# LambdaLabsML/distributed-training-guide

Hardware: NVIDIA H100
Metric: tokens/sec (device-timed, max over ranks) Llama-2-7B seq 4096 bf16 training (higher is better)
Workload: dtype bf16; 1 GPU; model=meta-llama/Llama-2-7b-hf, global_batch=1, seq_len=4096, parallelism=dp1 (ddp+zero1), optimizer=AdamW, bf16 parameters and states

## Files before the change

distributed_training_guide_b200/csrc/api.h:

```cpp
#pragma once
#include <cuda_runtime.h>
#include <cstdint>

namespace dtg {

unsigned long long launch_count();

enum class NormKind : int { kRms, kLn, kLn2 };
enum class NormRes : int { kNone, kAddBefore, kAddAfter };
constexpr int norm_grad_planes(NormKind k) { return k == NormKind::kRms ? 1 : k == NormKind::kLn ? 2 : 4; }
int norm_max_hidden(NormKind k);
struct NormFwdArgs {
  const void* x;
  const void* r;
  const void* w[2];
  const void* b[2];
  void* y[2];
  void* h;
  float* mean;
  float* rstd;
};
void norm_fwd(NormKind k, NormRes res, const NormFwdArgs& a, int T, int H, float eps, cudaStream_t s);
int norm_bwd_grid(NormKind k, int T, int H);
struct NormBwdArgs {
// ... 49 lines not shown
void adamw_flat(void* p, const void* g, void* m, void* v, long long n, float lr, float beta1, float beta2, float eps,
                float wd, int step, float grad_scale, bool state_fp32, cudaStream_t s);

void gemm_bf16(const void* A, const void* B, void* C, int M, int N, int K, long long lda, long long ldb, long long ldc,
               bool a_kmajor, bool b_kmajor, bool accumulate, int variant, cudaStream_t s, const void* bias = nullptr);

void gemm_fp8(const void* A, const void* B, void* C, int M, int N, int K, long long lda, long long ldb, long long ldc,
              bool a_e5m2, const float* scale_a, const float* scale_b, bool accumulate, int variant, cudaStream_t s,
              const void* bias = nullptr);

int gemm_max_active_clusters(int cg);
void gemm_bf16_dist(int mode, const void* const* a_srcs, const void* const* b_srcs, void* const* c_dsts, int M, int N,
                    int K, long long lda, long long ldb, long long ldc, bool b_kmajor, bool accumulate, int nranks,
                    int rank, int rows_per_peer, cudaStream_t s);

void gemm_bf16_bgather(const void* A, void* full_base, void* C, int M, int N, int K, long long lda, long long ldb,
                       long long ldc, bool b_kmajor, const void* const* shards, long long per_bytes, long long w_off,
                       long long w_bytes, uint32_t* counters, uint32_t target, int chunk_shift, uint32_t* const* pads,
                       int nranks, int rank, uint32_t bar_epoch, cudaStream_t s, const void* bias = nullptr);
void gemm_bf16_ag(const void* const* a_bufs, const void* B, void* C, int M, int N, int K, long long ldb, long long ldc,
                  bool b_kmajor, int nranks, int rank, int rows_per_peer, uint32_t* flags, uint32_t ag_epoch,
                  uint32_t* const* pads, uint32_t bar_epoch, int n_comm, cudaStream_t s, const void* bias = nullptr);

void fp8_amax(const void* x, long long R, int C, long long ld, float* amax, cudaStream_t s);
void fp8_cast_transpose(const void* x, long long ld, int R, int C, bool e5m2, const float* amax, void* out, void* out_t,
                        float* scale_inv, cudaStream_t s);

void attn_fwd(const void* qkv, void* o, float* lse, int B, int S, int nh, int nkv, float scale, cudaStream_t s,
              const int* doc_start = nullptr, int window = 0, int head_dim = 128);
void attn_fwd2(const void* qkv, void* o, float* lse, int B, int S, int nh, int nkv, float scale, cudaStream_t s,
               const int* doc_start = nullptr, int window = 0, int head_dim = 128);
void attn_bwd(const void* qkv, const void* o, const void* d_o, const float* lse, float* delta, float* dq_acc,
              void* dqkv, int B, int S, int nh, int nkv, float scale, int mode, cudaStream_t s,
              const int* doc_start = nullptr, int window = 0, int head_dim = 128);

}
```

distributed_training_guide_b200/csrc/attention_bind.cpp:

```cpp
#include <ATen/cuda/CUDAContext.h>
#include <c10/cuda/CUDAGuard.h>
#include <torch/extension.h>

#include <algorithm>
#include <cmath>
#include <cstdint>
#include <cstdlib>
#include <limits>

#include "api.h"
#include "comm_api.h"

namespace dtg {
namespace {
using torch::Tensor;

void check_heads_scale(int64_t nh, int64_t nkv, double scale) {
  TORCH_CHECK(nh >= 1 && nkv >= 1, "nh and nkv must be >= 1, got nh ", nh, ", nkv ", nkv);
  TORCH_CHECK(nh % nkv == 0, "nh must be a multiple of nkv, got nh ", nh, ", nkv ", nkv);
  const float s = (float)scale;
  TORCH_CHECK(std::isfinite(s) && s > 0.f, "scale must be finite and > 0, got ", scale);
}

bool aligned16(const Tensor& t) { return reinterpret_cast<uintptr_t>(t.data_ptr()) % 16 == 0; }
// ... 48 lines not shown
  return (int)std::min<int64_t>(*window, std::numeric_limits<int>::max());
}

int default_fwd_version() {
  static int v = -1;
  if (v < 0) {
    const char* e = getenv("DTG_ATTN_FWD");
    v = e ? atoi(e) : 2;
    if (v != 1 && v != 2) v = 2;
  }
  return v;
}

std::tuple<Tensor, Tensor> py_attn_fwd(const Tensor& qkv, int64_t nh, int64_t nkv, double scale, int64_t version,
                                       const c10::optional<Tensor>& doc_start, const c10::optional<int64_t>& window,
                                       int64_t head_dim) {
  check_qkv(qkv, nh, nkv, scale, head_dim);
  TORCH_CHECK(version >= 0 && version <= 2, "version must be 0 (default), 1 or 2, got ", version);
  const int* ds = doc_start_ptr(doc_start, qkv);
  const int win = window_arg(window);
  const c10::cuda::CUDAGuard guard(qkv.device());
  const int64_t B = qkv.size(0), S = qkv.size(1);
  Tensor o = torch::empty({B, S, nh, head_dim}, qkv.options());
  Tensor lse = torch::empty({B, nh, S}, qkv.options().dtype(at::kFloat));
  if (version == 0) version = default_fwd_version();
  auto fn = version == 1 ? dtg::attn_fwd : dtg::attn_fwd2;
  fn(qkv.data_ptr(), o.data_ptr(), lse.data_ptr<float>(), (int)B, (int)S, (int)nh, (int)nkv, (float)scale,
     at::cuda::getCurrentCUDAStream().stream(), ds, win, (int)head_dim);
  return {o, lse};
}

Tensor py_attn_bwd(const Tensor& d_o, const Tensor& qkv, const Tensor& o, const Tensor& lse, int64_t nh, int64_t nkv,
                   double scale, const c10::optional<Tensor>& trace, int64_t mode,
                   const c10::optional<Tensor>& doc_start, const c10::optional<int64_t>& window, int64_t head_dim) {
  check_qkv(qkv, nh, nkv, scale, head_dim);
  TORCH_CHECK(mode >= 0 && mode <= 2, "mode must be 0 (default), 1 or 2, got ", mode);
  const int* ds = doc_start_ptr(doc_start, qkv);
  const int win = window_arg(window);
  check_rows(o, "o", qkv, nh, head_dim);
  check_rows(d_o, "d_o", qkv, nh, head_dim);
  check_lse(lse, qkv, nh);
  float* tr = nullptr;
  if (trace.has_value() && trace->defined()) {
    TORCH_CHECK(trace->scalar_type() == at::kLong && trace->numel() >= 1024 && trace->is_contiguous() &&
                    trace->device() == qkv.device(),
                "trace must be a contiguous int64[1024] on the device of qkv");
    tr = reinterpret_cast<float*>(trace->data_ptr<int64_t>());
  }
  const c10::cuda::CUDAGuard guard(qkv.device());
  const int64_t B = qkv.size(0), S = qkv.size(1);
  Tensor dqkv = torch::empty_like(qkv);
  Tensor delta = torch::empty({B, nh, S}, qkv.options().dtype(at::kFloat));
  dtg::attn_bwd(qkv.data_ptr(), o.data_ptr(), d_o.data_ptr(), lse.data_ptr<float>(), delta.data_ptr<float>(), tr,
                dqkv.data_ptr(), (int)B, (int)S, (int)nh, (int)nkv, (float)scale, (int)mode,
                at::cuda::getCurrentCUDAStream().stream(), ds, win, (int)head_dim);
  return dqkv;
}
}

void bind_attention(pybind11::module_& m) {
  m.def("attn_fwd", &py_attn_fwd, pybind11::arg("qkv"), pybind11::arg("nh"), pybind11::arg("nkv"), pybind11::arg("scale"),
        pybind11::arg("version") = 0, pybind11::arg("doc_start") = pybind11::none(),
        pybind11::arg("window") = pybind11::none(), pybind11::arg("head_dim") = 128);
  m.def("attn_bwd", &py_attn_bwd, pybind11::arg("d_o"), pybind11::arg("qkv"), pybind11::arg("o"), pybind11::arg("lse"),
        pybind11::arg("nh"), pybind11::arg("nkv"), pybind11::arg("scale"), pybind11::arg("trace") = pybind11::none(),
        pybind11::arg("mode") = 0,
        pybind11::arg("doc_start") = pybind11::none(), pybind11::arg("window") = pybind11::none(),
        pybind11::arg("head_dim") = 128);
}
}
```

distributed_training_guide_b200/csrc/attention_bwd.cu:

```cuda
#include <cuda.h>

#include <cstdlib>

#include "api.h"
#include "attention_common.cuh"
#include "common.cuh"
#include "gemm_common.cuh"
#include "ptx.cuh"

namespace dtg {
using namespace ptx;

namespace bwd {
constexpr int R_HALF = 128 * 128;
constexpr int C_HALF = 64 * 128;
constexpr int Y_STAGES = 3;
constexpr float LOG2E = 1.4426950408889634f;
constexpr int THREADS = 256;
template <int D>
struct Layout {
  static constexpr int R_TILE = 128 * D * 2;
  static constexpr int C_TILE = 64 * D * 2;
  static constexpr int OFF_R1 = 0, OFF_R2 = R_TILE;
  static constexpr int OFF_Y = 2 * R_TILE;
  static constexpr int OFF_P = OFF_Y + Y_STAGES * 2 * C_TILE;
  static constexpr int OFF_DS = OFF_P + 128 * 128;
  static constexpr int OFF_BAR = OFF_DS + 128 * 128;
  static constexpr int SMEM_BYTES = OFF_BAR + 256 + 1024;
};
}

template <int D>
__global__ void attn_bwd_delta_kernel(const __nv_bfloat16* __restrict__ d_o, const __nv_bfloat16* __restrict__ o,
                                      float* __restrict__ delta, long long rows, int S, int nh) {
  const long long row = (blockIdx.x * (long long)blockDim.x + threadIdx.x) >> 5;
  const int lane = threadIdx.x & 31;
  if (row >= rows) return;
  const __nv_bfloat162* a = reinterpret_cast<const __nv_bfloat162*>(d_o + row * D) + lane * (D / 64);
  const __nv_bfloat162* b = reinterpret_cast<const __nv_bfloat162*>(o + row * D) + lane * (D / 64);
  float acc = 0.f;
#pragma unroll
  for (int i = 0; i < D / 64; ++i) {
    const float2 x = __bfloat1622float2(a[i]), y = __bfloat1622float2(b[i]);
    acc += x.x * y.x + x.y * y.y;
  }
  acc = warp_sum(acc);
  if (lane == 0) {
    const long long tok = row / nh;
    const int h = (int)(row % nh);
    const long long bb = tok / S, ss = tok % S;
    delta[(bb * nh + h) * S + ss] = acc;
  }
}

template <bool KV_MODE, bool TS, bool DOC, bool WIN, int D>
__global__ void __launch_bounds__(bwd::THREADS, 1)
attn_bwd_kernel(const __grid_constant__ CUtensorMap tm_qkv_r, const __grid_constant__ CUtensorMap tm_qkv_c,
                const __grid_constant__ CUtensorMap tm_do_r, const __grid_constant__ CUtensorMap tm_do_c,
                const float* __restrict__ lse, const float* __restrict__ delta, __nv_bfloat16* __restrict__ dqkv,
                int S, int nh, int nkv, float scale, int num_r_blocks, long long* __restrict__ trace,
                const int* __restrict__ doc_start, int window) {
  using namespace bwd;
  using L = Layout<D>;
  constexpr int R_TILE = L::R_TILE, C_TILE = L::C_TILE, OFF_R1 = L::OFF_R1, OFF_R2 = L::OFF_R2, OFF_Y = L::OFF_Y,
                OFF_P = L::OFF_P, OFF_DS = L::OFF_DS, OFF_BAR = L::OFF_BAR;
  const bool tracing = trace != nullptr && blockIdx.x == 0 && blockIdx.y == 0;
  extern __shared__ uint8_t smem_raw[];
  uint8_t* smem = reinterpret_cast<uint8_t*>((reinterpret_cast<uintptr_t>(smem_raw) + 1023) & ~uintptr_t(1023));
  uint64_t* bars = reinterpret_cast<uint64_t*>(smem + OFF_BAR);
  uint64_t* res_full = bars + 0;
  uint64_t* y_full = bars + 1;
  uint64_t* y_empty = bars + 5;

  const int warp = threadIdx.x >> 5, lane = threadIdx.x & 31, wg = threadIdx.x >> 7;
  const int group = nh / nkv;
  const int nht = nh + 2 * nkv;
  const int heads_r = KV_MODE ? nkv : nh;
  const int head_r = blockIdx.x % heads_r;
  const int batch = blockIdx.x / heads_r;
  const int r_block = KV_MODE ? (int)blockIdx.y : num_r_blocks - 1 - (int)blockIdx.y;
  const int R0 = r_block * 128;
  const int kv_head = KV_MODE ? head_r : head_r / group;
  int c_start = KV_MODE ? R0 / 64 : 0;
  int n_c = KV_MODE ? (S / 64 - c_start) : (R0 + 128) / 64;
  [[maybe_unused]] const int* ds_row = nullptr;
  [[maybe_unused]] int doc_bound = 0;
  if constexpr (DOC) {
    ds_row = doc_start + (long long)batch * S;
    if (KV_MODE) {
      int lo = c_start, hi = S / 64 - 1;
      while (lo < hi) {
        const int mid = (lo + hi + 1) >> 1;
        if (__ldg(ds_row + mid * 64) <= R0 + 127) lo = mid;
        else hi = mid - 1;
      }
      n_c = lo - c_start + 1;
      hi = c_start + n_c;
      lo = c_start;
      while (lo < hi) {
        const int mid = (lo + hi) >> 1;
        if (__ldg(ds_row + mid * 64 + 63) > R0) hi = mid;
        else lo = mid + 1;
      }
      doc_bound = lo;
    } else {
      c_start = min(max(__ldg(ds_row + R0) / 64, 0), n_c - 1);
      n_c -= c_start;
      doc_bound = __ldg(ds_row + R0 + 127);
    }
  }
  if constexpr (WIN) {
    if (KV_MODE) {
      n_c = min(n_c, min((R0 + 127 + window - 1) / 64, S / 64 - 1) - c_start + 1);
    } else {
      const int c_win = max(R0 - window + 1, 0) / 64;
      if (c_win > c_start) {
        n_c -= c_win - c_start;
        c_start = c_win;
      }
    }
  }
  const int n_iter = KV_MODE ? n_c * group : n_c;

  if (threadIdx.x == 0) {
    prefetch_tensormap(&tm_qkv_r);
    prefetch_tensormap(&tm_qkv_c);
    prefetch_tensormap(&tm_do_r);
    prefetch_tensormap(&tm_do_c);
    mbar_init(res_full, 1);
    for (int i = 0; i < Y_STAGES; ++i) {
      mbar_init(&y_full[i], 1);
      mbar_init(&y_empty[i], 2);
    }
    fence_barrier_init();
  }
  __syncthreads();

  auto issue_y = [&](int t) {
    const int st = t % Y_STAGES;
    const uint32_t ph = (uint32_t)((t / Y_STAGES) & 1);
    const int c = c_start + (KV_MODE ? t % n_c : t);
    const int C0 = c * 64;
    uint8_t* y1 = smem + OFF_Y + st * 2 * C_TILE;
    uint8_t* y2 = y1 + C_TILE;
    mbar_wait_mma(&y_empty[st], ph ^ 1);
    mbar_arrive_expect_tx(&y_full[st], 2 * C_TILE);
    if (KV_MODE) {
      const int qh = kv_head * group + t / n_c;
#pragma unroll
      for (int b = 0; b < D / 64; ++b) tma_load_4d(&tm_qkv_c, &y_full[st], y1 + b * C_HALF, 64 * b, qh, C0, batch);
#pragma unroll
      for (int b = 0; b < D / 64; ++b) tma_load_4d(&tm_do_c, &y_full[st], y2 + b * C_HALF, 64 * b, qh, C0, batch);
    } else {
#pragma unroll
      for (int b = 0; b < D / 64; ++b)
        tma_load_4d(&tm_qkv_c, &y_full[st], y1 + b * C_HALF, 64 * b, nh + kv_head, C0, batch);
#pragma unroll
      for (int b = 0; b < D / 64; ++b)
        tma_load_4d(&tm_qkv_c, &y_full[st], y2 + b * C_HALF, 64 * b, nh + nkv + kv_head, C0, batch);
    }
  };
// ... 42 lines not shown
        const long long idx = ((long long)batch * nh + head_r) * S + R0 + rl0 + 8 * h;
        lse_r[h] = lse[idx] * LOG2E;
        delta_r[h] = delta[idx];
        if constexpr (DOC) ds_r[h] = __ldg(ds_row + R0 + rl0 + 8 * h);
      }
    }
    if constexpr (WIN) {
#pragma unroll
      for (int h = 0; h < 2; ++h) {
        const int idx = R0 + rl0 + 8 * h;
        if constexpr (KV_MODE) ds_r[h] = DOC ? min(ds_r[h], idx + window) : idx + window;
        else ds_r[h] = max(ds_r[h], idx - window + 1);
      }
    }
    [[maybe_unused]] float acc_a[KV_MODE ? D / 2 : 1];
    float acc_b[D / 2];
#pragma unroll
    for (int i = 0; i < D / 2; ++i) {
      if constexpr (KV_MODE) acc_a[i] = 0.f;
      acc_b[i] = 0.f;
    }
    const uint32_t r1 = smem_u32(smem + OFF_R1) + (uint32_t)(half * 8192);
    const uint32_t r2 = smem_u32(smem + OFF_R2) + (uint32_t)(half * 8192);
    const uint32_t sp = smem_u32(smem + OFF_P) + (uint32_t)(half * 8192);
    const uint32_t sds = smem_u32(smem + OFF_DS) + (uint32_t)(half * 8192);
    mbar_wait_mma(res_full, 0);
    for (int t = 0; t < n_iter; ++t) {
      if (threadIdx.x == 0 && t + Y_STAGES - 1 < n_iter) issue_y(t + Y_STAGES - 1);
      const int ys = t % Y_STAGES;
      const int c = c_start + (KV_MODE ? t % n_c : t);
      const int C0 = c * 64;
      [[maybe_unused]] const float* lq = nullptr;
      [[maybe_unused]] const float* dq = nullptr;
      if (KV_MODE) {
        const int qh = kv_head * group + t / n_c;
        lq = lse + ((long long)batch * nh + qh) * S + C0;
        dq = delta + ((long long)batch * nh + qh) * S + C0;
      }
      mbar_wait_mma(&y_full[ys], (uint32_t)((t / Y_STAGES) & 1));
      const uint32_t y1 = smem_u32(smem + OFF_Y + ys * 2 * C_TILE), y2 = y1 + C_TILE;
      float sc[32], dp[32];
#pragma unroll
      for (int i = 0; i < 32; ++i) sc[i] = dp[i] = 0.f;
      wgmma_fence();
      fence_regs(sc);
      fence_regs(dp);
#pragma unroll
      for (int kk = 0; kk < D / 16; ++kk) {
        const uint32_t ra = (uint32_t)((kk >> 2) * R_HALF + (kk & 3) * 32);
        const uint32_t cb = (uint32_t)((kk >> 2) * C_HALF + (kk & 3) * 32);
        wgmma_m64n64k16_ss<0, 0>(sc, desc_kmajor_sw128(r1 + ra), desc_kmajor_sw128(y1 + cb), 1u);
      }
#pragma unroll
      for (int kk = 0; kk < D / 16; ++kk) {
        const uint32_t ra = (uint32_t)((kk >> 2) * R_HALF + (kk & 3) * 32);
        const uint32_t cb = (uint32_t)((kk >> 2) * C_HALF + (kk & 3) * 32);
        wgmma_m64n64k16_ss<0, 0>(dp, desc_kmajor_sw128(r2 + ra), desc_kmajor_sw128(y2 + cb), 1u);
      }
      wgmma_commit();
      wgmma_wait<0>();
      fence_regs(sc);
      fence_regs(dp);
      if (tr_thread && t < 64) trace[t * 8 + 0] = clock64();
      bool need_mask = KV_MODE ? (C0 < R0 + 127) : (C0 + 63 > R0);
      if constexpr (DOC) need_mask = need_mask || (KV_MODE ? c >= doc_bound : C0 < doc_bound);
      if constexpr (WIN) need_mask = need_mask || (KV_MODE ? C0 + 63 >= R0 + window : C0 < R0 + 128 - window);
#pragma unroll
      for (int i = 0; i < 32; ++i) {
        const int col = 8 * (i >> 2) + 2 * tq + (i & 1);
        const int h = (i >> 1) & 1;
        const int row = rl0 + 8 * h;
        float l2, dl;
        if constexpr (KV_MODE) {
          l2 = __ldg(lq + col) * LOG2E;
          dl = __ldg(dq + col);
        } else {
          l2 = lse_r[h];
          dl = delta_r[h];
        }
        float p = fast_exp2(fmaf(sc[i], sl2, -l2));
        if (need_mask) {
          bool ok = KV_MODE ? (C0 + col >= R0 + row) : (R0 + row >= C0 + col);
          if constexpr (DOC || WIN) ok = ok && (KV_MODE ? C0 + col < ds_r[h] : C0 + col >= ds_r[h]);
          p = ok ? p : 0.f;
        }
        sc[i] = p;
        dp[i] = p * (dp[i] - dl) * scale;
      }
      uint32_t pp[4][4], pd[4][4];
#pragma unroll
      for (int kk = 0; kk < 4; ++kk)
#pragma unroll
        for (int r = 0; r < 4; ++r) {
          pp[kk][r] = pack_bf16x2(sc[8 * kk + 2 * r], sc[8 * kk + 2 * r + 1]);
          pd[kk][r] = pack_bf16x2(dp[8 * kk + 2 * r], dp[8 * kk + 2 * r + 1]);
        }
      if (tr_thread && t < 64) trace[t * 8 + 1] = clock64();
      if constexpr (!TS) {
#pragma unroll
        for (int kk = 0; kk < 4; ++kk)
#pragma unroll
          for (int r = 0; r < 4; ++r) {
            const int row = rl0 + ((r & 1) ? 8 : 0);
            const int col = 16 * kk + ((r & 2) ? 8 : 0) + 2 * tq;
            const int off = row * 128 + (((col >> 3) ^ (row & 7)) << 4) + (col & 7) * 2;
            if (KV_MODE) *reinterpret_cast<uint32_t*>(smem + OFF_P + off) = pp[kk][r];
            *reinterpret_cast<uint32_t*>(smem + OFF_DS + off) = pd[kk][r];
          }
        fence_proxy_async();
        named_bar_sync(1 + half, 128);
      }
      wgmma_fence();
      if constexpr (KV_MODE) fence_regs(acc_a);
      fence_regs(acc_b);
      if constexpr (KV_MODE) {
#pragma unroll
        for (int kk = 0; kk < 4; ++kk) {
          const uint64_t db = desc_mnmajor_sw128(y2 + kk * 2048, C_HALF);
          if constexpr (TS) wgmma_bf16_rs<1>(acc_a, pp[kk], db, 1u);
          else wgmma_bf16_ss<0, 1>(acc_a, desc_kmajor_sw128(sp + kk * 32), db, 1u);
        }
      }
#pragma unroll
      for (int kk = 0; kk < 4; ++kk) {
        const uint64_t db = desc_mnmajor_sw128(y1 + kk * 2048, C_HALF);
        if constexpr (TS) wgmma_bf16_rs<1>(acc_b, pd[kk], db, 1u);
        else wgmma_bf16_ss<0, 1>(acc_b, desc_kmajor_sw128(sds + kk * 32), db, 1u);
      }
      wgmma_commit();
      wgmma_wait<0>();
      if constexpr (KV_MODE) fence_regs(acc_a);
      fence_regs(acc_b);
      if (signal) mbar_arrive(&y_empty[ys]);
      if constexpr (!TS) named_bar_sync(1 + half, 128);
      if (tr_thread && t < 64) trace[t * 8 + 3] = clock64();
    }
#pragma unroll
    for (int h = 0; h < 2; ++h) {
      const long long tok = (long long)batch * S + R0 + rl0 + 8 * h;
      auto write_row = [&](const float (&acc)[D / 2], int out_head) {
        __nv_bfloat16* dst = dqkv + (tok * nht + out_head) * (long long)D;
#pragma unroll
        for (int nb = 0; nb < D / 8; ++nb)
          *reinterpret_cast<__nv_bfloat162*>(dst + 8 * nb + 2 * tq) =
              __floats2bfloat162_rn(acc[4 * nb + 2 * h], acc[4 * nb + 2 * h + 1]);
      };
      if constexpr (KV_MODE) {
        write_row(acc_a, nh + nkv + kv_head);
        write_row(acc_b, nh + kv_head);
      } else {
        write_row(acc_b, head_r);
      }
    }
  }
}

template <bool TS, bool DOC, bool WIN, int D>
static void launch_attn_bwd(const CUtensorMap& tq_r, const CUtensorMap& tq_c, const CUtensorMap& td_r,
                            const CUtensorMap& td_c, const float* lse, const float* delta, void* dqkv, int B, int S,
                            int nh, int nkv, float scale, long long* trace, const int* doc_start, int window,
                            cudaStream_t s) {
  constexpr int smem = bwd::Layout<D>::SMEM_BYTES;
  static bool attr = false;
  if (!attr) {
    DTG_CUDA_CHECK(cudaFuncSetAttribute(attn_bwd_kernel<true, TS, DOC, WIN, D>,
                                        cudaFuncAttributeMaxDynamicSharedMemorySize, smem));
    DTG_CUDA_CHECK(cudaFuncSetAttribute(attn_bwd_kernel<false, TS, DOC, WIN, D>,
                                        cudaFuncAttributeMaxDynamicSharedMemorySize, smem));
    attr = true;
  }
  const int nblk = S / 128;
  attn_bwd_kernel<true, TS, DOC, WIN, D><<<dim3(B * nkv, nblk, 1), bwd::THREADS, smem, s>>>(
      tq_r, tq_c, td_r, td_c, lse, delta, (__nv_bfloat16*)dqkv, S, nh, nkv, scale, nblk, trace, doc_start, window);
  attn_bwd_kernel<false, TS, DOC, WIN, D><<<dim3(B * nh, nblk, 1), bwd::THREADS, smem, s>>>(
      tq_r, tq_c, td_r, td_c, lse, delta, (__nv_bfloat16*)dqkv, S, nh, nkv, scale, nblk, trace ? trace + 512 : nullptr,
      doc_start, window);
}

template <bool TS, int D>
static void dispatch_attn_bwd(const CUtensorMap& tq_r, const CUtensorMap& tq_c, const CUtensorMap& td_r,
                              const CUtensorMap& td_c, const float* lse, const float* delta, void* dqkv, int B, int S,
                              int nh, int nkv, float scale, long long* trace, const int* doc_start, int window,
                              cudaStream_t s) {
  if (window > 0 && window < S) {
    if (doc_start) launch_attn_bwd<TS, true, true, D>(tq_r, tq_c, td_r, td_c, lse, delta, dqkv, B, S, nh, nkv, scale, trace, doc_start, window, s);
    else launch_attn_bwd<TS, false, true, D>(tq_r, tq_c, td_r, td_c, lse, delta, dqkv, B, S, nh, nkv, scale, trace, nullptr, window, s);
  } else {
    if (doc_start) launch_attn_bwd<TS, true, false, D>(tq_r, tq_c, td_r, td_c, lse, delta, dqkv, B, S, nh, nkv, scale, trace, doc_start, 0, s);
    else launch_attn_bwd<TS, false, false, D>(tq_r, tq_c, td_r, td_c, lse, delta, dqkv, B, S, nh, nkv, scale, trace, nullptr, 0, s);
  }
}

void attn_bwd(const void* qkv, const void* o, const void* d_o, const float* lse, float* delta, float* trace_buf,
              void* dqkv, int B, int S, int nh, int nkv, float scale, int mode, cudaStream_t s,
              const int* doc_start, int window, int head_dim) {
  long long* trace = reinterpret_cast<long long*>(trace_buf);
  if (S % 128 != 0) throw std::runtime_error("attn_bwd: sequence length must be a multiple of 128");
  if (window < 0) throw std::runtime_error("attn_bwd: window must be >= 1 (0 = no window)");
  if (nh < 1 || nkv < 1 || nh % nkv != 0) throw std::runtime_error("attn_bwd: nh must be a positive multiple of nkv");
  if (head_dim != 64 && head_dim != 128) throw std::runtime_error("attn_bwd: head_dim must be 64 or 128");
  const CUtensorMap tq_r = make_tmap_heads(qkv, B, S, nh + 2 * nkv, 128, head_dim);
  const CUtensorMap tq_c = make_tmap_heads(qkv, B, S, nh + 2 * nkv, 64, head_dim);
  const CUtensorMap td_r = make_tmap_heads(d_o, B, S, nh, 128, head_dim);
  const CUtensorMap td_c = make_tmap_heads(d_o, B, S, nh, 64, head_dim);
  const long long rows = (long long)B * S * nh;
  const unsigned delta_blocks = (unsigned)((rows * 32 + 255) / 256);
  if (head_dim == 128)
    attn_bwd_delta_kernel<128><<<delta_blocks, 256, 0, s>>>((const __nv_bfloat16*)d_o, (const __nv_bfloat16*)o, delta,
                                                            rows, S, nh);
  else
    attn_bwd_delta_kernel<64><<<delta_blocks, 256, 0, s>>>((const __nv_bfloat16*)d_o, (const __nv_bfloat16*)o, delta,
                                                           rows, S, nh);
  static const bool ts_default = []() {
    const char* e = getenv("DTG_ATTN_BWD");
    return e ? e[0] != 's' : true;
  }();
  const bool ts = mode == 0 ? ts_default : mode == 2;
  if (head_dim == 128) {
    if (ts) dispatch_attn_bwd<true, 128>(tq_r, tq_c, td_r, td_c, lse, delta, dqkv, B, S, nh, nkv, scale, trace, doc_start, window, s);
    else dispatch_attn_bwd<false, 128>(tq_r, tq_c, td_r, td_c, lse, delta, dqkv, B, S, nh, nkv, scale, trace, doc_start, window, s);
  } else {
    if (ts) dispatch_attn_bwd<true, 64>(tq_r, tq_c, td_r, td_c, lse, delta, dqkv, B, S, nh, nkv, scale, trace, doc_start, window, s);
    else dispatch_attn_bwd<false, 64>(tq_r, tq_c, td_r, td_c, lse, delta, dqkv, B, S, nh, nkv, scale, trace, doc_start, window, s);
  }
  note_launch(3);
  DTG_LAUNCH_CHECK();
}

}
```

distributed_training_guide_b200/csrc/ptx.cuh:

```cuda
#pragma once
#include <cuda.h>
#include <cuda_bf16.h>
#include <cstdint>
#include <cstdio>

namespace dtg {
namespace ptx {

__device__ __forceinline__ uint32_t smem_u32(const void* p) { return (uint32_t)__cvta_generic_to_shared(p); }

__device__ __forceinline__ uint32_t lane_id() {
  uint32_t l;
  asm volatile("mov.u32 %0, %%laneid;" : "=r"(l));
  return l;
}

__device__ __forceinline__ bool elect_one() {
  uint32_t pred = 0;
  asm volatile(
      "{\n\t"
      ".reg .pred P1;\n\t"
      "elect.sync _|P1, 0xffffffff;\n\t"
      "selp.u32 %0, 1, 0, P1;\n\t"
      "}\n"
// ... 129 lines not shown
      "cp.async.bulk.tensor.2d.shared::cluster.global.mbarrier::complete_tx::bytes.multicast::cluster [%0], [%1, {%3, %4}], "
      "[%2], %5;"
      :
      : "r"(smem_u32(smem)), "l"(reinterpret_cast<uint64_t>(m)), "r"(smem_u32(bar)), "r"(c0), "r"(c1), "h"(cta_mask)
      : "memory");
}
__device__ __forceinline__ void tma_load_3d(const CUtensorMap* m, uint64_t* bar, void* smem, int c0, int c1, int c2) {
  asm volatile(
      "cp.async.bulk.tensor.3d.shared::cluster.global.mbarrier::complete_tx::bytes [%0], [%1, {%3, %4, %5}], [%2];"
      :
      : "r"(smem_u32(smem)), "l"(reinterpret_cast<uint64_t>(m)), "r"(smem_u32(bar)), "r"(c0), "r"(c1), "r"(c2)
      : "memory");
}
__device__ __forceinline__ void tma_load_4d(const CUtensorMap* m, uint64_t* bar, void* smem, int c0, int c1, int c2,
                                            int c3) {
  asm volatile(
      "cp.async.bulk.tensor.4d.shared::cluster.global.mbarrier::complete_tx::bytes [%0], [%1, {%3, %4, %5, %6}], [%2];"
      :
      : "r"(smem_u32(smem)), "l"(reinterpret_cast<uint64_t>(m)), "r"(smem_u32(bar)), "r"(c0), "r"(c1), "r"(c2),
        "r"(c3)
      : "memory");
}
__device__ __forceinline__ void tma_store_2d(const CUtensorMap* m, const void* smem, int c0, int c1) {
  asm volatile("cp.async.bulk.tensor.2d.global.shared::cta.bulk_group [%0, {%2, %3}], [%1];"
               :
               : "l"(reinterpret_cast<uint64_t>(m)), "r"(smem_u32(smem)), "r"(c0), "r"(c1)
               : "memory");
}
__device__ __forceinline__ void tma_store_4d(const CUtensorMap* m, const void* smem, int c0, int c1, int c2, int c3) {
  asm volatile("cp.async.bulk.tensor.4d.global.shared::cta.bulk_group [%0, {%2, %3, %4, %5}], [%1];"
               :
               : "l"(reinterpret_cast<uint64_t>(m)), "r"(smem_u32(smem)), "r"(c0), "r"(c1), "r"(c2), "r"(c3)
               : "memory");
}
__device__ __forceinline__ void tma_store_commit() { asm volatile("cp.async.bulk.commit_group;" ::: "memory"); }
template <int N>
__device__ __forceinline__ void tma_store_wait_read() {
  asm volatile("cp.async.bulk.wait_group.read %0;" ::"n"(N) : "memory");
}
template <int N>
__device__ __forceinline__ void tma_store_wait() {
  asm volatile("cp.async.bulk.wait_group %0;" ::"n"(N) : "memory");
}

__device__ __forceinline__ void bulk_load_g2s(void* smem, const void* gsrc, uint32_t bytes, uint64_t* bar) {
  asm volatile("cp.async.bulk.shared::cluster.global.mbarrier::complete_tx::bytes [%0], [%1], %2, [%3];"
               :
               : "r"(smem_u32(smem)), "l"(gsrc), "r"(bytes), "r"(smem_u32(bar))
               : "memory");
}
__device__ __forceinline__ void bulk_store_s2g(void* gdst, const void* smem, uint32_t bytes) {
  asm volatile("cp.async.bulk.global.shared::cta.bulk_group [%0], [%1], %2;" ::"l"(gdst), "r"(smem_u32(smem)), "r"(bytes)
               : "memory");
}
__device__ __forceinline__ void bulk_commit_group() { asm volatile("cp.async.bulk.commit_group;" ::: "memory"); }
template <int N>
__device__ __forceinline__ void bulk_wait_group_read() {
  asm volatile("cp.async.bulk.wait_group.read %0;" ::"n"(N) : "memory");
}
template <int N>
__device__ __forceinline__ void bulk_wait_group() {
  asm volatile("cp.async.bulk.wait_group %0;" ::"n"(N) : "memory");
}
__device__ __forceinline__ void fence_proxy_async_all() { asm volatile("fence.proxy.async;" ::: "memory"); }
__device__ __forceinline__ void st_release_gpu(uint32_t* p, uint32_t v) {
  asm volatile("st.release.gpu.global.u32 [%0], %1;" ::"l"(p), "r"(v) : "memory");
// ... 206 lines not shown
```

Baseline: 12070 tokens/s.

## Store dS in the KV backward pass and compute dQ from it

The attention backward KV pass now also writes the masked dS tiles to a global workspace through TMA stores with an L2 evict-first hint. A new dQ kernel streams those stored dS tiles together with K tiles through a 3-stage mbarrier pipeline and does a single GEMM per tile. This replaces the old dQ pass, which recomputed QK^T, the softmax probabilities and dP. The cost is a large extra write and read of dS per layer, roughly half a GB at this shape, plus an extra workspace allocation. By default the path is used when head_dim is 128 and the workspace fits under a 4 GiB cap.

```diff
diff --git a/distributed_training_guide_b200/csrc/api.h b/distributed_training_guide_b200/csrc/api.h
--- a/distributed_training_guide_b200/csrc/api.h
+++ b/distributed_training_guide_b200/csrc/api.h
@@ -105,6 +105,9 @@
                const int* doc_start = nullptr, int window = 0, int head_dim = 128);
 void attn_bwd(const void* qkv, const void* o, const void* d_o, const float* lse, float* delta, float* dq_acc,
               void* dqkv, int B, int S, int nh, int nkv, float scale, int mode, cudaStream_t s,
-              const int* doc_start = nullptr, int window = 0, int head_dim = 128);
+              const int* doc_start = nullptr, int window = 0, int head_dim = 128, void* ds_workspace = nullptr);
+constexpr long long kAttnBwdDsCapBytes = 4LL << 30;
+long long attn_bwd_ds_bytes(int B, int S, int nh);
+int attn_bwd_dq_path(int B, int S, int nh, int head_dim, int dq);
 
 }
diff --git a/distributed_training_guide_b200/csrc/attention_bind.cpp b/distributed_training_guide_b200/csrc/attention_bind.cpp
--- a/distributed_training_guide_b200/csrc/attention_bind.cpp
+++ b/distributed_training_guide_b200/csrc/attention_bind.cpp
@@ -104,9 +104,11 @@
 
 Tensor py_attn_bwd(const Tensor& d_o, const Tensor& qkv, const Tensor& o, const Tensor& lse, int64_t nh, int64_t nkv,
                    double scale, const c10::optional<Tensor>& trace, int64_t mode,
-                   const c10::optional<Tensor>& doc_start, const c10::optional<int64_t>& window, int64_t head_dim) {
+                   const c10::optional<Tensor>& doc_start, const c10::optional<int64_t>& window, int64_t head_dim,
+                   int64_t dq, const c10::optional<Tensor>& workspace) {
   check_qkv(qkv, nh, nkv, scale, head_dim);
   TORCH_CHECK(mode >= 0 && mode <= 2, "mode must be 0 (default), 1 or 2, got ", mode);
+  TORCH_CHECK(dq >= 0 && dq <= 2, "dq must be 0 (default), 1 (recompute) or 2 (stored dS), got ", dq);
   const int* ds = doc_start_ptr(doc_start, qkv);
   const int win = window_arg(window);
   check_rows(o, "o", qkv, nh, head_dim);
@@ -123,9 +125,22 @@
   const int64_t B = qkv.size(0), S = qkv.size(1);
   Tensor dqkv = torch::empty_like(qkv);
   Tensor delta = torch::empty({B, nh, S}, qkv.options().dtype(at::kFloat));
+  Tensor ws;
+  if (dtg::attn_bwd_dq_path((int)B, (int)S, (int)nh, (int)head_dim, (int)dq) == 2) {
+    const int64_t bytes = dtg::attn_bwd_ds_bytes((int)B, (int)S, (int)nh);
+    if (workspace.has_value() && workspace->defined()) {
+      ws = *workspace;
+      TORCH_CHECK(ws.is_contiguous() && ws.device() == qkv.device() && ws.nbytes() >= (size_t)bytes &&
+                      reinterpret_cast<uintptr_t>(ws.data_ptr()) % 16 == 0,
+                  "workspace must be a contiguous 16-byte aligned tensor of at least ", bytes,
+                  " bytes on the device of qkv");
+    } else {
+      ws = torch::empty({bytes}, qkv.options().dtype(at::kByte));
+    }
+  }
   dtg::attn_bwd(qkv.data_ptr(), o.data_ptr(), d_o.data_ptr(), lse.data_ptr<float>(), delta.data_ptr<float>(), tr,
                 dqkv.data_ptr(), (int)B, (int)S, (int)nh, (int)nkv, (float)scale, (int)mode,
-                at::cuda::getCurrentCUDAStream().stream(), ds, win, (int)head_dim);
+                at::cuda::getCurrentCUDAStream().stream(), ds, win, (int)head_dim, ws.defined() ? ws.data_ptr() : nullptr);
   return dqkv;
 }
 }
@@ -138,6 +153,12 @@
         pybind11::arg("nh"), pybind11::arg("nkv"), pybind11::arg("scale"), pybind11::arg("trace") = pybind11::none(),
         pybind11::arg("mode") = 0,
         pybind11::arg("doc_start") = pybind11::none(), pybind11::arg("window") = pybind11::none(),
-        pybind11::arg("head_dim") = 128);
+        pybind11::arg("head_dim") = 128,
+        pybind11::arg("dq") = 0,
+        pybind11::arg("workspace") = pybind11::none());
+  m.def("attn_bwd_ds_bytes", &dtg::attn_bwd_ds_bytes, pybind11::arg("B"), pybind11::arg("S"), pybind11::arg("nh"));
+  m.def("attn_bwd_dq_path", &dtg::attn_bwd_dq_path, pybind11::arg("B"), pybind11::arg("S"), pybind11::arg("nh"),
+        pybind11::arg("head_dim") = 128, pybind11::arg("dq") = 0);
+  m.attr("ATTN_BWD_DS_CAP_BYTES") = dtg::kAttnBwdDsCapBytes;
 }
 }
diff --git a/distributed_training_guide_b200/csrc/attention_bwd.cu b/distributed_training_guide_b200/csrc/attention_bwd.cu
--- a/distributed_training_guide_b200/csrc/attention_bwd.cu
+++ b/distributed_training_guide_b200/csrc/attention_bwd.cu
@@ -28,6 +28,40 @@
   static constexpr int OFF_BAR = OFF_DS + 128 * 128;
   static constexpr int SMEM_BYTES = OFF_BAR + 256 + 1024;
 };
+
+constexpr int DS_TILE = 128 * 128;
+constexpr int DQ_STAGES = 3;
+constexpr int MAX_KEY_BLOCKS = 512;
+template <int D>
+struct DqLayout {
+  static constexpr int K_TILE = 128 * D * 2;
+  static constexpr int STAGE = K_TILE + 2 * DS_TILE;
+  static constexpr int OFF_VIS = DQ_STAGES * STAGE;
+  static constexpr int OFF_BAR = OFF_VIS + MAX_KEY_BLOCKS;
+  static constexpr int SMEM_BYTES = OFF_BAR + 2 * DQ_STAGES * 8 + 1024;
+};
+
+template <bool DOC, bool WIN>
+__device__ __forceinline__ int kv_query_blocks(int R0, int S, const int* ds_row, int window) {
+  const int c_start = R0 / 64;
+  int n_c = S / 64 - c_start;
+  if constexpr (DOC) {
+    int lo = c_start, hi = S / 64 - 1;
+    while (lo < hi) {
+      const int mid = (lo + hi + 1) >> 1;
+      if (__ldg(ds_row + mid * 64) <= R0 + 127) lo = mid;
+      else hi = mid - 1;
+    }
+    n_c = lo - c_start + 1;
+  }
+  if constexpr (WIN) n_c = min(n_c, min((R0 + 127 + window - 1) / 64, S / 64 - 1) - c_start + 1);
+  return n_c;
+}
+
+__device__ __forceinline__ int ds_tile_row(int bh, int r, int c, int S) {
+  const int nR = S / 128;
+  return (bh * nR * (nR + 1) + r * (S / 64) - r * (r - 1) + (c - 2 * r)) * 128;
+}
 }
 
 template <int D>
@@ -53,15 +87,18 @@
   }
 }
 
-template <bool KV_MODE, bool TS, bool DOC, bool WIN, int D>
+template <bool KV_MODE, bool TS, bool DOC, bool WIN, int D, bool STORE = false>
 __global__ void __launch_bounds__(bwd::THREADS, 1)
 attn_bwd_kernel(const __grid_constant__ CUtensorMap tm_qkv_r, const __grid_constant__ CUtensorMap tm_qkv_c,
                 const __grid_constant__ CUtensorMap tm_do_r, const __grid_constant__ CUtensorMap tm_do_c,
+                const __grid_constant__ CUtensorMap tm_ds,
                 const float* __restrict__ lse, const float* __restrict__ delta, __nv_bfloat16* __restrict__ dqkv,
                 int S, int nh, int nkv, float scale, int num_r_blocks, long long* __restrict__ trace,
                 const int* __restrict__ doc_start, int window) {
   using namespace bwd;
   using L = Layout<D>;
+  static_assert(KV_MODE || !STORE, "only the KV pass stores dS^T");
+  constexpr bool store_ds = STORE;
   constexpr int R_TILE = L::R_TILE, C_TILE = L::C_TILE, OFF_R1 = L::OFF_R1, OFF_R2 = L::OFF_R2, OFF_Y = L::OFF_Y,
                 OFF_P = L::OFF_P, OFF_DS = L::OFF_DS, OFF_BAR = L::OFF_BAR;
   const bool tracing = trace != nullptr && blockIdx.x == 0 && blockIdx.y == 0;
@@ -85,18 +122,11 @@
   int n_c = KV_MODE ? (S / 64 - c_start) : (R0 + 128) / 64;
   [[maybe_unused]] const int* ds_row = nullptr;
   [[maybe_unused]] int doc_bound = 0;
+  if constexpr (DOC) ds_row = doc_start + (long long)batch * S;
+  if (KV_MODE) n_c = kv_query_blocks<DOC, WIN>(R0, S, ds_row, window);
   if constexpr (DOC) {
-    ds_row = doc_start + (long long)batch * S;
     if (KV_MODE) {
-      int lo = c_start, hi = S / 64 - 1;
-      while (lo < hi) {
-        const int mid = (lo + hi + 1) >> 1;
-        if (__ldg(ds_row + mid * 64) <= R0 + 127) lo = mid;
-        else hi = mid - 1;
-      }
-      n_c = lo - c_start + 1;
-      hi = c_start + n_c;
-      lo = c_start;
+      int hi = c_start + n_c, lo = c_start;
       while (lo < hi) {
         const int mid = (lo + hi) >> 1;
         if (__ldg(ds_row + mid * 64 + 63) > R0) hi = mid;
@@ -110,9 +140,7 @@
     }
   }
   if constexpr (WIN) {
-    if (KV_MODE) {
-      n_c = min(n_c, min((R0 + 127 + window - 1) / 64, S / 64 - 1) - c_start + 1);
-    } else {
+    if (!KV_MODE) {
       const int c_win = max(R0 - window + 1, 0) / 64;
       if (c_win > c_start) {
         n_c -= c_win - c_start;
@@ -127,6 +155,7 @@
     prefetch_tensormap(&tm_qkv_c);
     prefetch_tensormap(&tm_do_r);
     prefetch_tensormap(&tm_do_c);
+    if (KV_MODE && store_ds) prefetch_tensormap(&tm_ds);
     mbar_init(res_full, 1);
     for (int i = 0; i < Y_STAGES; ++i) {
       mbar_init(&y_full[i], 1);
@@ -235,10 +264,12 @@
       const int C0 = c * 64;
       [[maybe_unused]] const float* lq = nullptr;
       [[maybe_unused]] const float* dq = nullptr;
+      [[maybe_unused]] int ds_row0 = 0;
       if (KV_MODE) {
         const int qh = kv_head * group + t / n_c;
         lq = lse + ((long long)batch * nh + qh) * S + C0;
         dq = delta + ((long long)batch * nh + qh) * S + C0;
+        ds_row0 = ds_tile_row(batch * nh + qh, r_block, c, S) + half * 64;
       }
       mbar_wait_mma(&y_full[ys], (uint32_t)((t / Y_STAGES) & 1));
       const uint32_t y1 = smem_u32(smem + OFF_Y + ys * 2 * C_TILE), y2 = y1 + C_TILE;
@@ -282,13 +313,15 @@
           dl = delta_r[h];
         }
         float p = fast_exp2(fmaf(sc[i], sl2, -l2));
+        bool ok = true;
         if (need_mask) {
-          bool ok = KV_MODE ? (C0 + col >= R0 + row) : (R0 + row >= C0 + col);
+          ok = KV_MODE ? (C0 + col >= R0 + row) : (R0 + row >= C0 + col);
           if constexpr (DOC || WIN) ok = ok && (KV_MODE ? C0 + col < ds_r[h] : C0 + col >= ds_r[h]);
           p = ok ? p : 0.f;
         }
         sc[i] = p;
         dp[i] = p * (dp[i] - dl) * scale;
+        if (STORE && !ok) dp[i] = 0.f;
       }
       uint32_t pp[4][4], pd[4][4];
 #pragma unroll
@@ -299,7 +332,7 @@
           pd[kk][r] = pack_bf16x2(dp[8 * kk + 2 * r], dp[8 * kk + 2 * r + 1]);
         }
       if (tr_thread && t < 64) trace[t * 8 + 1] = clock64();
-      if constexpr (!TS) {
+      auto stage = [&](int off_ds, bool with_p) {
 #pragma unroll
         for (int kk = 0; kk < 4; ++kk)
 #pragma unroll
@@ -307,11 +340,22 @@
             const int row = rl0 + ((r & 1) ? 8 : 0);
             const int col = 16 * kk + ((r & 2) ? 8 : 0) + 2 * tq;
             const int off = row * 128 + (((col >> 3) ^ (row & 7)) << 4) + (col & 7) * 2;
-            if (KV_MODE) *reinterpret_cast<uint32_t*>(smem + OFF_P + off) = pp[kk][r];
-            *reinterpret_cast<uint32_t*>(smem + OFF_DS + off) = pd[kk][r];
+            if (with_p) *reinterpret_cast<uint32_t*>(smem + OFF_P + off) = pp[kk][r];
+            *reinterpret_cast<uint32_t*>(smem + off_ds + off) = pd[kk][r];
           }
         fence_proxy_async();
+      };
+      auto store_warp_rows = [&](int off_ds) {
+        if (lane == 0) {
+          const int w16 = (warp & 3) * 16;
+          tma_store_2d_hint(&tm_ds, smem + off_ds + half * 8192 + w16 * 128, 0, ds_row0 + w16, l2_evict_first_policy());
+          bulk_commit_group();
+        }
+      };
+      if constexpr (!TS) {
+        stage(OFF_DS, KV_MODE);
         named_bar_sync(1 + half, 128);
+        if (KV_MODE && store_ds) store_warp_rows(OFF_DS);
       }
       wgmma_fence();
       if constexpr (KV_MODE) fence_regs(acc_a);
@@ -331,13 +375,25 @@
         else wgmma_bf16_ss<0, 1>(acc_b, desc_kmajor_sw128(sds + kk * 32), db, 1u);
       }
       wgmma_commit();
+      if (TS && KV_MODE && store_ds) {
+        const int off_ds = (t & 1) ? OFF_P : OFF_DS;
+        if (lane == 0) bulk_wait_group_read<1>();
+        __syncwarp();
+        stage(off_ds, false);
+        __syncwarp();
+        store_warp_rows(off_ds);
+      }
       wgmma_wait<0>();
       if constexpr (KV_MODE) fence_regs(acc_a);
       fence_regs(acc_b);
       if (signal) mbar_arrive(&y_empty[ys]);
-      if constexpr (!TS) named_bar_sync(1 + half, 128);
+      if constexpr (!TS) {
+        if (KV_MODE && store_ds && lane == 0) bulk_wait_group_read<0>();
+        named_bar_sync(1 + half, 128);
+      }
       if (tr_thread && t < 64) trace[t * 8 + 3] = clock64();
     }
+    if (KV_MODE && store_ds && lane == 0) bulk_wait_group<0>();
 #pragma unroll
     for (int h = 0; h < 2; ++h) {
       const long long tok = (long long)batch * S + R0 + rl0 + 8 * h;
@@ -358,45 +414,171 @@
   }
 }
 
+template <bool DOC, bool WIN, int D>
+__global__ void __launch_bounds__(bwd::THREADS, 1)
+attn_bwd_dq_kernel(const __grid_constant__ CUtensorMap tm_qkv_r, const __grid_constant__ CUtensorMap tm_ds,
+                   __nv_bfloat16* __restrict__ dqkv, int S, int nh, int nkv, const int* __restrict__ doc_start,
+                   int window) {
+  using namespace bwd;
+  using L = DqLayout<D>;
+  extern __shared__ uint8_t smem_raw[];
+  uint8_t* smem = reinterpret_cast<uint8_t*>((reinterpret_cast<uintptr_t>(smem_raw) + 1023) & ~uintptr_t(1023));
+  uint8_t* vis = smem + L::OFF_VIS;
+  uint64_t* full = reinterpret_cast<uint64_t*>(smem + L::OFF_BAR);
+  uint64_t* empty = full + DQ_STAGES;
+
+  const int warp = threadIdx.x >> 5, lane = threadIdx.x & 31, wg = threadIdx.x >> 7;
+  const int group = nh / nkv, nht = nh + 2 * nkv;
+  const int qh = blockIdx.x % nh, batch = blockIdx.x / nh;
+  const int kv_head = qh / group;
+  const int j = S / 128 - 1 - (int)blockIdx.y;
+  const int bh = batch * nh + qh;
+  [[maybe_unused]] const int* ds_row = DOC ? doc_start + (long long)batch * S : nullptr;
+  for (int r = threadIdx.x; r <= j; r += THREADS) {
+    const int end = 2 * r + kv_query_blocks<DOC, WIN>(r * 128, S, ds_row, window);
+    vis[r] = (uint8_t)((2 * j < end ? 1 : 0) | (2 * j + 1 < end ? 2 : 0));
+  }
+  if (threadIdx.x == 0) {
+    prefetch_tensormap(&tm_qkv_r);
+    prefetch_tensormap(&tm_ds);
+    for (int i = 0; i < DQ_STAGES; ++i) {
+      mbar_init(&full[i], 1);
+      mbar_init(&empty[i], 2);
+    }
+    fence_barrier_init();
+  }
+  __syncthreads();
+
+  int r_issue = 0, n_issued = 0;
+  auto issue_next = [&]() {
+    while (r_issue <= j && vis[r_issue] == 0) ++r_issue;
+    if (r_issue > j) return;
+    const int m = vis[r_issue];
+    const int st = n_issued % DQ_STAGES;
+    const uint32_t ph = (uint32_t)((n_issued / DQ_STAGES) & 1);
+    uint8_t* kt = smem + st * L::STAGE;
+    mbar_wait_mma(&empty[st], ph ^ 1);
+    mbar_arrive_expect_tx(&full[st], L::K_TILE + __popc(m) * DS_TILE);
+#pragma unroll
+    for (int b = 0; b < D / 64; ++b)
+      tma_load_4d(&tm_qkv_r, &full[st], kt + b * R_HALF, 64 * b, nh + kv_head, r_issue * 128, batch);
+#pragma unroll
+    for (int h = 0; h < 2; ++h)
+      if (m >> h & 1) {
+        const int row = ds_tile_row(bh, r_issue, 2 * j + h, S);
+        uint8_t* dt = kt + L::K_TILE + h * DS_TILE;
+        const uint64_t once = l2_evict_first_policy();
+        tma_load_2d_hint(&tm_ds, &full[st], dt, 0, row, once);
+        tma_load_2d_hint(&tm_ds, &full[st], dt + DS_TILE / 2, 0, row + 64, once);
+      }
+    ++r_issue;
+    ++n_issued;
+  };
+  if (threadIdx.x == 0)
+    for (int i = 0; i < DQ_STAGES - 1; ++i) issue_next();
+
+  const int g = lane >> 2, tq = lane & 3;
+  float acc[D / 2];
+#pragma unroll
+  for (int i = 0; i < D / 2; ++i) acc[i] = 0.f;
+  int t = 0;
+  for (int r = 0; r <= j; ++r) {
+    const int m = vis[r];
+    if (m == 0) continue;
+    if (threadIdx.x == 0) issue_next();
+    const int st = t % DQ_STAGES;
+    mbar_wait_mma(&full[st], (uint32_t)((t / DQ_STAGES) & 1));
+    if (m >> wg & 1) {
+      const uint32_t kt = smem_u32(smem + st * L::STAGE);
+      const uint32_t dt = kt + L::K_TILE + wg * DS_TILE;
+      wgmma_fence();
+      fence_regs(acc);
+#pragma unroll
+      for (int kk = 0; kk < 8; ++kk)
+        wgmma_bf16_ss<1, 1>(acc, desc_mnmajor_sw128(dt + kk * 2048, C_HALF), desc_mnmajor_sw128(kt + kk * 2048, R_HALF),
+                            1u);
+      wgmma_commit();
+      wgmma_wait<0>();
+      fence_regs(acc);
+    }
+    if ((threadIdx.x & 127) == 0) mbar_arrive(&empty[st]);
+    ++t;
+  }
+  const int rl0 = wg * 64 + (warp & 3) * 16 + g;
+#pragma unroll
+  for (int h = 0; h < 2; ++h) {
+    const long long tok = (long long)batch * S + j * 128 + rl0 + 8 * h;
+    __nv_bfloat16* dst = dqkv + (tok * nht + qh) * (long long)D;
+#pragma unroll
+    for (int nb = 0; nb < D / 8; ++nb)
+      *reinterpret_cast<__nv_bfloat162*>(dst + 8 * nb + 2 * tq) =
+          __floats2bfloat162_rn(acc[4 * nb + 2 * h], acc[4 * nb + 2 * h + 1]);
+  }
+}
+
 template <bool TS, bool DOC, bool WIN, int D>
 static void launch_attn_bwd(const CUtensorMap& tq_r, const CUtensorMap& tq_c, const CUtensorMap& td_r,
-                            const CUtensorMap& td_c, const float* lse, const float* delta, void* dqkv, int B, int S,
-                            int nh, int nkv, float scale, long long* trace, const int* doc_start, int window,
-                            cudaStream_t s) {
+                            const CUtensorMap& td_c, const CUtensorMap& tds_st, const CUtensorMap& tds_ld, bool store_ds, const float* lse,
+                            const float* delta, void* dqkv, int B, int S, int nh, int nkv, float scale, long long* trace,
+                            const int* doc_start, int window, cudaStream_t s) {
   constexpr int smem = bwd::Layout<D>::SMEM_BYTES;
+  constexpr int smem_dq = bwd::DqLayout<D>::SMEM_BYTES;
   static bool attr = false;
   if (!attr) {
     DTG_CUDA_CHECK(cudaFuncSetAttribute(attn_bwd_kernel<true, TS, DOC, WIN, D>,
                                         cudaFuncAttributeMaxDynamicSharedMemorySize, smem));
+    DTG_CUDA_CHECK(cudaFuncSetAttribute(attn_bwd_kernel<true, TS, DOC, WIN, D, true>,
+                                        cudaFuncAttributeMaxDynamicSharedMemorySize, smem));
     DTG_CUDA_CHECK(cudaFuncSetAttribute(attn_bwd_kernel<false, TS, DOC, WIN, D>,
                                         cudaFuncAttributeMaxDynamicSharedMemorySize, smem));
+    DTG_CUDA_CHECK(cudaFuncSetAttribute(attn_bwd_dq_kernel<DOC, WIN, D>,
+                                        cudaFuncAttributeMaxDynamicSharedMemorySize, smem_dq));
     attr = true;
   }
   const int nblk = S / 128;
-  attn_bwd_kernel<true, TS, DOC, WIN, D><<<dim3(B * nkv, nblk, 1), bwd::THREADS, smem, s>>>(
-      tq_r, tq_c, td_r, td_c, lse, delta, (__nv_bfloat16*)dqkv, S, nh, nkv, scale, nblk, trace, doc_start, window);
-  attn_bwd_kernel<false, TS, DOC, WIN, D><<<dim3(B * nh, nblk, 1), bwd::THREADS, smem, s>>>(
-      tq_r, tq_c, td_r, td_c, lse, delta, (__nv_bfloat16*)dqkv, S, nh, nkv, scale, nblk, trace ? trace + 512 : nullptr,
-      doc_start, window);
+  if (store_ds) {
+    attn_bwd_kernel<true, TS, DOC, WIN, D, true><<<dim3(B * nkv, nblk, 1), bwd::THREADS, smem, s>>>(
+        tq_r, tq_c, td_r, td_c, tds_st, lse, delta, (__nv_bfloat16*)dqkv, S, nh, nkv, scale, nblk, trace, doc_start,
+        window);
+    attn_bwd_dq_kernel<DOC, WIN, D><<<dim3(B * nh, nblk, 1), bwd::THREADS, smem_dq, s>>>(
+        tq_r, tds_ld, (__nv_bfloat16*)dqkv, S, nh, nkv, doc_start, window);
+  } else {
+    attn_bwd_kernel<true, TS, DOC, WIN, D><<<dim3(B * nkv, nblk, 1), bwd::THREADS, smem, s>>>(
+        tq_r, tq_c, td_r, td_c, tds_st, lse, delta, (__nv_bfloat16*)dqkv, S, nh, nkv, scale, nblk, trace, doc_start,
+        window);
+    attn_bwd_kernel<false, TS, DOC, WIN, D><<<dim3(B * nh, nblk, 1), bwd::THREADS, smem, s>>>(
+        tq_r, tq_c, td_r, td_c, tds_st, lse, delta, (__nv_bfloat16*)dqkv, S, nh, nkv, scale, nblk,
+        trace ? trace + 512 : nullptr, doc_start, window);
+  }
 }
 
 template <bool TS, int D>
 static void dispatch_attn_bwd(const CUtensorMap& tq_r, const CUtensorMap& tq_c, const CUtensorMap& td_r,
-                              const CUtensorMap& td_c, const float* lse, const float* delta, void* dqkv, int B, int S,
-                              int nh, int nkv, float scale, long long* trace, const int* doc_start, int window,
-                              cudaStream_t s) {
+                              const CUtensorMap& td_c, const CUtensorMap& tds_st, const CUtensorMap& tds_ld, bool store_ds, const float* lse,
+                              const float* delta, void* dqkv, int B, int S, int nh, int nkv, float scale,
+                              long long* trace, const int* doc_start, int window, cudaStream_t s) {
   if (window > 0 && window < S) {
-    if (doc_start) launch_attn_bwd<TS, true, true, D>(tq_r, tq_c, td_r, td_c, lse, delta, dqkv, B, S, nh, nkv, scale, trace, doc_start, window, s);
-    else launch_attn_bwd<TS, false, true, D>(tq_r, tq_c, td_r, td_c, lse, delta, dqkv, B, S, nh, nkv, scale, trace, nullptr, window, s);
+    if (doc_start) launch_attn_bwd<TS, true, true, D>(tq_r, tq_c, td_r, td_c, tds_st, tds_ld, store_ds, lse, delta, dqkv, B, S, nh, nkv, scale, trace, doc_start, window, s);
+    else launch_attn_bwd<TS, false, true, D>(tq_r, tq_c, td_r, td_c, tds_st, tds_ld, store_ds, lse, delta, dqkv, B, S, nh, nkv, scale, trace, nullptr, window, s);
   } else {
-    if (doc_start) launch_attn_bwd<TS, true, false, D>(tq_r, tq_c, td_r, td_c, lse, delta, dqkv, B, S, nh, nkv, scale, trace, doc_start, 0, s);
-    else launch_attn_bwd<TS, false, false, D>(tq_r, tq_c, td_r, td_c, lse, delta, dqkv, B, S, nh, nkv, scale, trace, nullptr, 0, s);
-  }
+    if (doc_start) launch_attn_bwd<TS, true, false, D>(tq_r, tq_c, td_r, td_c, tds_st, tds_ld, store_ds, lse, delta, dqkv, B, S, nh, nkv, scale, trace, doc_start, 0, s);
+    else launch_attn_bwd<TS, false, false, D>(tq_r, tq_c, td_r, td_c, tds_st, tds_ld, store_ds, lse, delta, dqkv, B, S, nh, nkv, scale, trace, nullptr, 0, s);
+  }
+}
+
+long long attn_bwd_ds_bytes(int B, int S, int nh) {
+  const long long nR = S / 128;
+  return (long long)B * nh * nR * (nR + 1) * bwd::DS_TILE;
+}
+
+int attn_bwd_dq_path(int B, int S, int nh, int head_dim, int dq) {
+  if (dq == 1 || dq == 2) return dq;
+  return head_dim == 128 && attn_bwd_ds_bytes(B, S, nh) <= kAttnBwdDsCapBytes ? 2 : 1;
 }
 
 void attn_bwd(const void* qkv, const void* o, const void* d_o, const float* lse, float* delta, float* trace_buf,
               void* dqkv, int B, int S, int nh, int nkv, float scale, int mode, cudaStream_t s,
-              const int* doc_start, int window, int head_dim) {
+              const int* doc_start, int window, int head_dim, void* ds_workspace) {
   long long* trace = reinterpret_cast<long long*>(trace_buf);
   if (S % 128 != 0) throw std::runtime_error("attn_bwd: sequence length must be a multiple of 128");
   if (window < 0) throw std::runtime_error("attn_bwd: window must be >= 1 (0 = no window)");
@@ -406,6 +588,15 @@
   const CUtensorMap tq_c = make_tmap_heads(qkv, B, S, nh + 2 * nkv, 64, head_dim);
   const CUtensorMap td_r = make_tmap_heads(d_o, B, S, nh, 128, head_dim);
   const CUtensorMap td_c = make_tmap_heads(d_o, B, S, nh, 64, head_dim);
+  const bool store_ds = ds_workspace != nullptr;
+  CUtensorMap tds_st{}, tds_ld{};
+  if (store_ds) {
+    const long long rows = attn_bwd_ds_bytes(B, S, nh) / 128;
+    if (S / 128 > bwd::MAX_KEY_BLOCKS || rows >= (1LL << 31))
+      throw std::runtime_error("attn_bwd: the stored-dS path needs S <= 65536 and a workspace below 256 GiB");
+    tds_st = make_tmap_2d(ds_workspace, 64, (uint64_t)rows, 128, 64, 16);
+    tds_ld = make_tmap_2d(ds_workspace, 64, (uint64_t)rows, 128, 64, 64);
+  }
   const long long rows = (long long)B * S * nh;
   const unsigned delta_blocks = (unsigned)((rows * 32 + 255) / 256);
   if (head_dim == 128)
@@ -420,11 +611,11 @@
   }();
   const bool ts = mode == 0 ? ts_default : mode == 2;
   if (head_dim == 128) {
-    if (ts) dispatch_attn_bwd<true, 128>(tq_r, tq_c, td_r, td_c, lse, delta, dqkv, B, S, nh, nkv, scale, trace, doc_start, window, s);
-    else dispatch_attn_bwd<false, 128>(tq_r, tq_c, td_r, td_c, lse, delta, dqkv, B, S, nh, nkv, scale, trace, doc_start, window, s);
+    if (ts) dispatch_attn_bwd<true, 128>(tq_r, tq_c, td_r, td_c, tds_st, tds_ld, store_ds, lse, delta, dqkv, B, S, nh, nkv, scale, trace, doc_start, window, s);
+    else dispatch_attn_bwd<false, 128>(tq_r, tq_c, td_r, td_c, tds_st, tds_ld, store_ds, lse, delta, dqkv, B, S, nh, nkv, scale, trace, doc_start, window, s);
   } else {
-    if (ts) dispatch_attn_bwd<true, 64>(tq_r, tq_c, td_r, td_c, lse, delta, dqkv, B, S, nh, nkv, scale, trace, doc_start, window, s);
-    else dispatch_attn_bwd<false, 64>(tq_r, tq_c, td_r, td_c, lse, delta, dqkv, B, S, nh, nkv, scale, trace, doc_start, window, s);
+    if (ts) dispatch_attn_bwd<true, 64>(tq_r, tq_c, td_r, td_c, tds_st, tds_ld, store_ds, lse, delta, dqkv, B, S, nh, nkv, scale, trace, doc_start, window, s);
+    else dispatch_attn_bwd<false, 64>(tq_r, tq_c, td_r, td_c, tds_st, tds_ld, store_ds, lse, delta, dqkv, B, S, nh, nkv, scale, trace, doc_start, window, s);
   }
   note_launch(3);
   DTG_LAUNCH_CHECK();
diff --git a/distributed_training_guide_b200/csrc/ptx.cuh b/distributed_training_guide_b200/csrc/ptx.cuh
--- a/distributed_training_guide_b200/csrc/ptx.cuh
+++ b/distributed_training_guide_b200/csrc/ptx.cuh
@@ -185,6 +185,25 @@
                :
                : "l"(reinterpret_cast<uint64_t>(m)), "r"(smem_u32(smem)), "r"(c0), "r"(c1), "r"(c2), "r"(c3)
                : "memory");
+}
+__device__ __forceinline__ uint64_t l2_evict_first_policy() {
+  uint64_t p;
+  asm volatile("createpolicy.fractional.L2::evict_first.b64 %0, 1.0;" : "=l"(p));
+  return p;
+}
+__device__ __forceinline__ void tma_store_2d_hint(const CUtensorMap* m, const void* smem, int c0, int c1, uint64_t policy) {
+  asm volatile("cp.async.bulk.tensor.2d.global.shared::cta.bulk_group.L2::cache_hint [%0, {%2, %3}], [%1], %4;"
+               :
+               : "l"(reinterpret_cast<uint64_t>(m)), "r"(smem_u32(smem)), "r"(c0), "r"(c1), "l"(policy)
+               : "memory");
+}
+__device__ __forceinline__ void tma_load_2d_hint(const CUtensorMap* m, uint64_t* bar, void* smem, int c0, int c1,
+                                                 uint64_t policy) {
+  asm volatile(
+      "cp.async.bulk.tensor.2d.shared::cluster.global.mbarrier::complete_tx::bytes.L2::cache_hint [%0], [%1, {%3, %4}], [%2], %5;"
+      :
+      : "r"(smem_u32(smem)), "l"(reinterpret_cast<uint64_t>(m)), "r"(smem_u32(bar)), "r"(c0), "r"(c1), "l"(policy)
+      : "memory");
 }
 __device__ __forceinline__ void tma_store_commit() { asm volatile("cp.async.bulk.commit_group;" ::: "memory"); }
 template <int N>
```

New measurement: 12180 tokens/s (median of 6 runs). Within noise of the previous version (+0.9%).
